# Pose-Group/FAMI-Pose

Measured on AMD Instinct MI355X. Metric: train clips/sec (5-frame 384x288 HRNet-W48), higher is better.
Workload: dtype f32

## Files before the change

### fami-pose_amd/csrc/conv.hip

```cpp
#include "common.h"
#include <type_traits>
#include <string.h>

#include "conv_epi.h"
#include "conv_pair.h"
extern "C" int fami_conv2d_fwd_bnin_ok(int N, int H, int W, int Ci, int Co);
extern "C" int fami_dcn_tune(int mode);
extern "C" int fami_bn_tune_small(long elems);
extern "C" void fami_conv_stem_tune(int on);
int fami_pair_launch(const PairCapture& c, hipStream_t s);
int fami_try_conv_stem1(int half_kind, const void* x, const void* wp, const float* bias, void* y, int N, int H, int W, int Ci, int Co,
                        int kh, int kw, int stride, int pad, int dil, int NTt, int relu, int accumulate, int out_f32, hipStream_t s,
                        const char* name, const EpiBN& epi);


struct ConvArgs {
  EpiBN e;
  int emode;
  const float* x;
  const float* wp;
  float* y;
  const float* bias;
  const float* addend;
  int N, Hi, Wi, Ci, Ho, Wo, Co;
// ... 1713 lines not shown
      for (int nt = 0; nt < NT; ++nt)
#pragma unroll
        for (int r = 0; r < 4; ++r) acc[mt][nt][r] += mine[((mt * NT + nt) * 4 + r) * 64];
  }
  if (!active) return;
  float* slabp = p.part + ((long)slab * taps + tap) * p.Ci * p.Co;
#pragma unroll
  for (int mt = 0; mt < MT; ++mt)
#pragma unroll
    for (int r = 0; r < 4; ++r) {
      const int cci = (cib * MT + mt) * 16 + kq * 4 + r;
#pragma unroll
      for (int nt = 0; nt < NT; ++nt) {
        const int cco = (cob * NT + nt) * 16 + c16;
        slabp[(long)cci * p.Co + cco] = acc[mt][nt][r];
      }
    }
}

__device__ __forceinline__ void reduce_taps_body(const float* __restrict__ part, float* __restrict__ dw, int Co, int Ci,
                                                 int taps, int psplit, int accumulate, int bid, float* sm ) {
  const long n = (long)taps * Ci * Co;
  const int o = threadIdx.x & 63, g = threadIdx.x >> 6;
  const long i = (long)bid * 64 + o;
  float s0 = 0.f, s1 = 0.f;
  if (i < n) {
    int k = g;
    for (; k + 16 < psplit; k += 32) {
      s0 += part[(long)k * n + i];
      s1 += part[(long)(k + 16) * n + i];
    }
    if (k < psplit) s0 += part[(long)k * n + i];
  }
  sm[threadIdx.x] = s0 + s1;
  __syncthreads();
  if (g == 0 && i < n) {
    float s = 0.f;
#pragma unroll
    for (int q = 0; q < 16; ++q) s += sm[q * 64 + o];
    const int co = (int)(i % Co);
    const long r = i / Co;
    const int ci = (int)(r % Ci), tap = (int)(r / Ci);
    float* d = dw + ((long)co * Ci + ci) * taps + tap;
    *d = accumulate ? *d + s : s;
  }
}
__global__ __launch_bounds__(1024) void wgrad_reduce_taps_kernel(const float* __restrict__ part,
                                                                 float* __restrict__ dw, int Co, int Ci, int taps,
                                                                 int psplit, int accumulate) {
  __shared__ float sm[1024];
  reduce_taps_body(part, dw, Co, Ci, taps, psplit, accumulate, blockIdx.x, sm);
}

__device__ __forceinline__ void reduce_taps4_body(const float* __restrict__ part, float* __restrict__ dw, int Co, int Ci,
                                                  int taps, int psplit, int accumulate, int sg, int bid, f32x4* sm ) {
  const int SG = 1 << sg, cols = 256 >> sg;
  const int o = threadIdx.x & (cols - 1), g = threadIdx.x >> (8 - sg);
  const long n4 = (long)taps * Ci * Co / 4;
  const long i = (long)bid * cols + o;
  const f32x4 z = {0.f, 0.f, 0.f, 0.f};
  f32x4 s0 = z, s1 = z, s2 = z, s3 = z;
  if (i < n4) {
    const f32x4* p4 = reinterpret_cast<const f32x4*>(part) + i;
    int k = g;
    for (; k + 7 * SG < psplit; k += 8 * SG) {
      const f32x4 v0 = p4[(long)k * n4], v1 = p4[(long)(k + SG) * n4], v2 = p4[(long)(k + 2 * SG) * n4],
                  v3 = p4[(long)(k + 3 * SG) * n4], v4 = p4[(long)(k + 4 * SG) * n4], v5 = p4[(long)(k + 5 * SG) * n4],
                  v6 = p4[(long)(k + 6 * SG) * n4], v7 = p4[(long)(k + 7 * SG) * n4];
      s0 += v0; s1 += v1; s2 += v2; s3 += v3;
      s0 += v4; s1 += v5; s2 += v6; s3 += v7;
    }
    for (; k + 3 * SG < psplit; k += 4 * SG) {
      s0 += p4[(long)k * n4];
      s1 += p4[(long)(k + SG) * n4];
      s2 += p4[(long)(k + 2 * SG) * n4];
      s3 += p4[(long)(k + 3 * SG) * n4];
    }
    for (; k < psplit; k += SG) s0 += p4[(long)k * n4];
  }
  sm[threadIdx.x] = (s0 + s1) + (s2 + s3);
  __syncthreads();
  if (g == 0 && i < n4) {
    f32x4 t = sm[o];
    for (int q = 1; q < SG; ++q) t += sm[q * cols + o];
    const long e = i * 4;
    const int co = (int)(e % Co);
    const long r = e / Co;
    const int ci = (int)(r % Ci), tap = (int)(r / Ci);
#pragma unroll
    for (int u = 0; u < 4; ++u) {
      float* d = dw + ((long)(co + u) * Ci + ci) * taps + tap;
      *d = accumulate ? *d + t[u] : t[u];
    }
  }
}
__global__ __launch_bounds__(256) void wgrad_reduce_taps4_kernel(const float* __restrict__ part, float* __restrict__ dw,
                                                                 int Co, int Ci, int taps, int psplit, int accumulate,
                                                                 int sg) {
  __shared__ f32x4 sm[256];
  reduce_taps4_body(part, dw, Co, Ci, taps, psplit, accumulate, sg, blockIdx.x, sm);
}

static void launch_reduce_taps(const float* part, float* dw, int Co, int Ci, int taps, int psplit, int accumulate,
                               hipStream_t s);

__device__ __forceinline__ void reduce_plain_body(const float* __restrict__ part, float* __restrict__ dw, long n,
                                                  int psplit, int accumulate, int bid, float* sm ) {
  const int o = threadIdx.x & 63, g = threadIdx.x >> 6;
  const long i = (long)bid * 64 + o;
  float s = 0.f;
  if (i < n)
    for (int k = g; k < psplit; k += 4) s += part[(long)k * n + i];
  sm[threadIdx.x] = s;
  __syncthreads();
  if (g == 0 && i < n) {
    s = sm[o] + sm[64 + o] + sm[128 + o] + sm[192 + o];
    dw[i] = accumulate ? dw[i] + s : s;
  }
}
__global__ __launch_bounds__(256) void wgrad_reduce_kernel(const float* __restrict__ part, float* __restrict__ dw,
                                                           long n, int psplit, int accumulate) {
  __shared__ float sm[256];
  reduce_plain_body(part, dw, n, psplit, accumulate, blockIdx.x, sm);
}

struct ReduceDesc {
  const float* part;
  float* dw;
  int Co, Ci, taps, psplit, accumulate, kind, sg, blocks;
};
#define FAMI_REDUCE_BATCH 16
struct ReduceBatch { ReduceDesc d[FAMI_REDUCE_BATCH]; };
__global__ __launch_bounds__(1024) void wgrad_reduce_batch_kernel(ReduceBatch b) {
  __shared__ f32x4 sm[256];
  const ReduceDesc& d = b.d[blockIdx.y];
  if ((int)blockIdx.x >= d.blocks) return;
  if (d.kind == 2) {
    reduce_taps_body(d.part, d.dw, d.Co, d.Ci, d.taps, d.psplit, d.accumulate, blockIdx.x, reinterpret_cast<float*>(sm));
    return;
  }
  if (threadIdx.x >= 256) return;
  if (d.kind == 1) reduce_taps4_body(d.part, d.dw, d.Co, d.Ci, d.taps, d.psplit, d.accumulate, d.sg, blockIdx.x, sm);
  else reduce_plain_body(d.part, d.dw, (long)d.Co * d.Ci * d.taps, d.psplit, d.accumulate, blockIdx.x, reinterpret_cast<float*>(sm));
}

typedef short s16x4 __attribute__((ext_vector_type(4)));
typedef __attribute__((address_space(3))) s16x4 lds_s16x4;

struct WgradLdsArgs {
  const void* x;
  const void* dy;
  float* part;
  int N, H, W, Ci, Co, P;
  int chunk;
  int nsub;
  int ciBlocks, coBlocks;
  int CiB, CoB;
  int xrow, yrow;
  int xbytes;
  int xcd;
};

template <typename H, int CIT, int COT>
__global__ __launch_bounds__(256) void conv_wgrad_h_kernel(WgradLdsArgs p) {
  typedef typename H16<H>::x8 hx8;
  extern __shared__ __attribute__((aligned(16))) char smem[];
  constexpr int NPW = (CIT * 9 + 3) / 4;
  const int tid = threadIdx.x, lane = tid & 63;
  const int wave = __builtin_amdgcn_readfirstlane(tid >> 6);
  const int l16 = lane & 15, kq = lane >> 4;
  const int rsel = l16 >> 2, piece = l16 & 3;
  int g, byl;
  xcd_tile(p.xcd, g, byl);
  const int cob = byl % p.coBlocks, cib = byl / p.coBlocks;
  const int halo = p.W + 1;
  char* xt = smem;
  char* yt = smem + p.xbytes;
  char* zrow = yt + p.chunk * p.yrow;

  int pci[NPW], ptap[NPW];
#pragma unroll
  for (int i = 0; i < NPW; ++i) {
    const int q = wave + 4 * i;
    const bool ok = q < CIT * 9;
    pci[i] = ok ? q / 9 : 0;
    ptap[i] = ok ? q % 9 : -1;
  }
  f32x4 acc[NPW][COT];
#pragma unroll
  for (int i = 0; i < NPW; ++i)
#pragma unroll
    for (int c = 0; c < COT; ++c) acc[i][c] = f32x4{0.f, 0.f, 0.f, 0.f};
  const int HW = p.H * p.W;

  for (int sub = 0; sub < p.nsub; ++sub) {
  const int p0 = (g * p.nsub + sub) * p.chunk;
// ... 267 lines not shown

template <typename T>
constexpr int storage_kind() { return std::is_same<T, float>::value ? 2 : (std::is_same<T, f16_t>::value ? 1 : 0); }

static bool wgrad_lin_ok(int H, int W, int Ci, int Co, int kh, int kw, int stride, int pad, int dil) {
  return stride == 1 && 2 * pad == dil * (kh - 1) && 2 * pad == dil * (kw - 1) && kh * kw > 1 && kh * kw <= 9 && W >= 4 &&
         Ci % 16 == 0 && Co % 16 == 0;
}
static bool geom_ok(int kh, int kw, int stride, int pad, int dil) {
  return kh >= 1 && kw >= 1 && kh <= 7 && kw <= 7 && (stride == 1 || stride == 2) && pad >= 0 && dil >= 1;
}
static inline int out_dim(int i, int k, int stride, int pad, int dil) {
  return (i + 2 * pad - dil * (k - 1) - 1) / stride + 1;
}
static int conv_args_check(const char* nm, bool ptrs, int N, int H, int W, int Ci, int Co, int kh, int kw, int stride, int pad,
                           int dil) {
  FAMI_REQUIRE(ptrs && N > 0 && H > 0 && W > 0 && Ci > 0 && Co > 0, nm, "bad argument");
  if (!geom_ok(kh, kw, stride, pad, dil)) {
    fami_set_error(nm, "unsupported geometry");
    return FAMI_ESHAPE;
  }
  return FAMI_OK;
}
template <typename Args>
static int conv_geometry(Args& a, const char* nm, int mode, int N, int H, int W, int Ci, int Co, int kh, int kw, int stride,
                         int pad, int dil, int esize, int kchunk) {
  const int Hc = out_dim(H, kh, stride, pad, dil), Wc = out_dim(W, kw, stride, pad, dil);
  a.N = N;
  a.Hi = mode ? Hc : H; a.Wi = mode ? Wc : W; a.Ci = mode ? Co : Ci;
  a.Ho = mode ? H : Hc; a.Wo = mode ? W : Wc; a.Co = mode ? Ci : Co;
  a.kh = kh; a.kw = kw; a.sh = stride == 2 ? 1 : 0; a.pad = pad; a.dil = dil;
  a.KC = fami_cdiv(a.Ci, kchunk); a.NTt = fami_cdiv(a.Co, 16);
  const long P = (long)N * a.Ho * a.Wo;
  const long xb = (long)N * a.Hi * a.Wi * a.Ci * esize, wb = (long)kh * kw * a.KC * a.NTt * 1024;
  FAMI_REQUIRE(P > 0 && P < (1L << 31) && xb < (1L << 31) && wb < (1L << 31), nm, "tensor >= 2 GiB");
  a.P = (int)P; a.x_bytes = (unsigned)xb; a.wp_bytes = (unsigned)wb;
  return FAMI_OK;
}

static thread_local ReduceDesc* g_defer = nullptr;
static ReduceDesc reduce_desc_taps(const float* part, float* dw, int Co, int Ci, int taps, int psplit, int accumulate) {
  ReduceDesc d;
  d.part = part; d.dw = dw; d.Co = Co; d.Ci = Ci; d.taps = taps; d.psplit = psplit; d.accumulate = accumulate;
  const long n = (long)Co * Ci * taps;
  if (Co % 4 == 0 && (reinterpret_cast<uintptr_t>(part) & 15) == 0) {
    int sg = 0;
    while (sg < 4 && (8 << sg) <= psplit) ++sg;
    d.kind = 1; d.sg = sg; d.blocks = fami_cdiv(n / 4, 256 >> sg);
  } else {
    d.kind = 2; d.sg = 0; d.blocks = fami_cdiv(n, 64);
  }
  return d;
}
static void launch_reduce_taps(const float* part, float* dw, int Co, int Ci, int taps, int psplit, int accumulate,
                               hipStream_t s) {
  const ReduceDesc d = reduce_desc_taps(part, dw, Co, Ci, taps, psplit, accumulate);
  if (g_defer) {
    *g_defer = d;
    return;
  }
  if (d.kind == 1)
    hipLaunchKernelGGL(wgrad_reduce_taps4_kernel, dim3(d.blocks), dim3(256), 0, s, part, dw, Co, Ci, taps, psplit, accumulate, d.sg);
  else
    hipLaunchKernelGGL(wgrad_reduce_taps_kernel, dim3(d.blocks), dim3(1024), 0, s, part, dw, Co, Ci, taps, psplit, accumulate);
}
static void launch_reduce_plain(const float* part, float* dw, int Co, int Ci, int taps, int psplit, int accumulate,
                                hipStream_t s) {
  const long n = (long)Co * Ci * taps;
  if (g_defer) {
    ReduceDesc d;
    d.part = part; d.dw = dw; d.Co = Co; d.Ci = Ci; d.taps = taps; d.psplit = psplit; d.accumulate = accumulate;
    d.kind = 0; d.sg = 0; d.blocks = fami_cdiv(n, 64);
    *g_defer = d;
    return;
  }
  hipLaunchKernelGGL(wgrad_reduce_kernel, dim3(fami_cdiv(n, 64)), dim3(256), 0, s, part, dw, n, psplit, accumulate);
}
template <typename Call>
static int with_deferred_reduce(const char* nm, long* desc_out, Call&& wgrad) {
  ReduceDesc d;
  d.part = nullptr;
  g_defer = &d;
  const int rc = wgrad();
  g_defer = nullptr;
  if (rc != FAMI_OK) return rc;
  FAMI_REQUIRE(d.part, nm, "no reduce recorded");
  memcpy(desc_out, &d, sizeof(d));
  return FAMI_OK;
}
template <typename Dgrad, typename Wgrad>
static int bwd_pair_run(const char* nm, long* desc_out, hipStream_t s, Dgrad&& dgrad, Wgrad&& wgrad) {
  PairCapture pc;
  pc.a.kind = pc.b.kind = 0;
  fami_pair_capture() = &pc;
  int rc = dgrad();
  if (rc == FAMI_OK) rc = with_deferred_reduce(nm, desc_out, wgrad);
  fami_pair_capture() = nullptr;
  if (rc != FAMI_OK) return rc;
  const int pr = fami_pair_launch(pc, s);
  FAMI_REQUIRE(pr >= 0, nm, "a recorded launch has no kernel instance");
  FAMI_CHECK_LAUNCH(nm);
  return FAMI_OK;
}

struct WgradPlan { int MT, NT, ciBlocks, coBlocks, psplit, chunk, pertap, w8; long P; };
static WgradPlan wgrad_plan(int N, int H, int W, int Ci, int Co, int kh, int kw, int stride, int pad, int dil, int w8 = 0) {
  WgradPlan q;
  const int Ho = out_dim(H, kh, stride, pad, dil), Wo = out_dim(W, kw, stride, pad, dil);
  q.P = (long)N * Ho * Wo;
  q.MT = pick_small(fami_cdiv(Ci, 16));
  q.NT = pick_small(fami_cdiv(Co, 16));
  if (g_wgrad_mt > 0 && g_wgrad_mt <= q.MT) q.MT = g_wgrad_mt;
  q.ciBlocks = fami_cdiv(fami_cdiv(Ci, 16), q.MT);
  q.coBlocks = fami_cdiv(fami_cdiv(Co, 16), q.NT);
// ... 682 lines not shown
                               epi_bwd_stats(slots, Ci, z, yrelu, mean, invstd, gamma, beta, relu));
}
template <typename HT>
static int bwd_pair_h(const char* nm, const HT* x, const HT* dy, const HT* wpd, HT* dx, float* dw, float* workspace, long ws_bytes,
                      int N, int H, int W, int Ci, int Co, int kh, int kw, int stride, int pad, int dil, int acc_dx, int acc_dw,
                      long* desc_out, const HT* z, const HT* yrelu, const float* mean, const float* invstd, const float* gamma,
                      const float* beta, int relu, void* slots, hipStream_t s) {
  FAMI_REQUIRE(desc_out, nm, "null descriptor");
  EpiBN e = epi_none();
  if (slots) {
    FAMI_REQUIRE(epi_bwd_stats_ok(z, yrelu, mean, invstd, gamma, beta, relu), nm, "bad argument");
    e = epi_bwd_stats(slots, Ci, z, yrelu, mean, invstd, gamma, beta, relu);
  }
  return bwd_pair_run(
      nm, desc_out, s,
      [&] { return conv_dgrad_h_impl<HT>(nm, dy, wpd, dx, N, H, W, Ci, Co, kh, kw, stride, pad, dil, acc_dx, s, e); },
      [&] { return wgrad_h_impl<HT>(nm, x, dy, dw, workspace, ws_bytes, N, H, W, Ci, Co, kh, kw, stride, pad, dil, acc_dw, s); });
}

extern "C" {

int fami_conv_tune(int mt, int nt, int ks) {
  g_force_mt = mt; g_force_nt = nt; g_force_ks = ks;
  return FAMI_OK;
}
int fami_conv_tune_lds(int on) {
  if (on == 9000 || on == 9001) {
    fami_conv_stem_tune(on - 9000);
    return FAMI_OK;
  }
  if (on < 0) fami_conv_stem_tune(-1);
  if (on == 10 || on == 11 || on == 20 || on == 21 || on == 30 || on == 31 || (on >= 40 && on <= 42) || (on >= 52 && on <= 54) || (on >= 60 && on <= 62) || on >= 100) {
    fami_conv_t4_tune(on);
    return FAMI_OK;
  }
  g_use_lds = on < 0 ? -1 : (on ? 1 : 0);
  g_lds_sim = on == 2;
  if (on < 0) fami_conv_t4_tune(-1);
  return FAMI_OK;
}
int fami_conv_tune_wgrad_lds(int on) {
  if (on >= 30000) {
    fami_wgrad_s3_tune(on - 30000);
    return FAMI_OK;
  }
  if (on >= 20000) {
    fami_wgrad16_tune(on - 20000);
    return FAMI_OK;
  }
  if (on >= 1000) {
    g_wgrad_ps = on - 1000;
    return FAMI_OK;
  }
  if (on >= 50 && on <= 54) {
    g_wgrad_lin = on - 50;
    return FAMI_OK;
  }
  if (on >= 100) {
    g_wgrad_mt = on - 100;
    return FAMI_OK;
  }
  if (on < 0) {
    fami_wgrad16_tune(-1);
    fami_wgrad_s3_tune(-1);
    g_wgrad_lds = 1;
    g_wgrad_lds_f32 = 2;
    g_wgrad_nsub = 2;
    g_wgrad_lin = 1;
    return FAMI_OK;
  }
  g_wgrad_lds = on ? 1 : 0;
  g_wgrad_lds_f32 = on ? 1 : 0;
  if (on > 1) g_wgrad_nsub = on - 1;
  return FAMI_OK;
}
int fami_conv_tune_xcd(int mode) {
  g_xcd = mode < 0 ? -1 : (mode & 1);
  g_xcd_w = mode < 0 ? 1 : ((mode >> 1) & 1);
  return FAMI_OK;
}
int fami_conv_tune_stages(int stages) {
  if (stages == 120 || stages == 121) {
    g_prio = stages - 120;
    return FAMI_OK;
  }
  if (stages == 110 || stages == 111) {
    g_par = stages - 110;
    return FAMI_OK;
  }
  if (stages == 100 || stages == 101) {
    g_lin_conv = stages - 100;
    return FAMI_OK;
  }
  g_stages = (stages >= 2 && stages <= 4) ? stages : 0;
  return FAMI_OK;
}
int fami_tune_reset(void) {
  fami_conv_tune(0, 0, 0);
  fami_conv_tune_lds(-1);
  fami_conv_tune_wgrad_lds(-1);
  fami_conv_tune_xcd(-1);
  g_stages = 0; g_prio = 0; g_lin_conv = 1; g_par = 1;
  g_wgrad_ps = 0; g_wgrad_mt = 0;
  fami_dcn_tune(-1);
  fami_bn_tune_small(-1);
  return FAMI_OK;
}
int fami_tune_defaults(int f32_split) {
  if (f32_split >= 0) {
    fami_conv_t4_default_split(f32_split);
    fami_wgrad_s3_default(f32_split);
  }
  return fami_tune_reset();
}

long fami_packed_weight_elems(int Co, int Ci, int kh, int kw, int mode) {
  const int kd = mode == 0 ? Ci : Co, nd = mode == 0 ? Co : Ci;
  return pack16_elems(kd, nd, kh * kw) + pack32_elems(kd, nd, kh * kw) + fami_split_image_elems(kd, nd, kh * kw);
}

int fami_pack_conv_weight_f32(const float* w_oihw, float* wp, int Co, int Ci, int kh, int kw, int mode,
// ... 77 lines not shown
  }
  if (kh == kw) {
    const long nl = fami_wgrad16_slabs(N, H, W, Ci, Co, kh, stride, pad, dil) * Co * Ci * kh * kw * (long)sizeof(float);
    if (nl > need) need = nl;
  }
  if (kh == 3 && kw == 3 && stride == 1 && pad == 1 && dil == 1) {
    const long nl = fami_wgrad_s3_slabs(N, H, W, Ci, Co) * Co * Ci * 9 * (long)sizeof(float);
    if (nl > need) need = nl;
  }
  return need;
}

int fami_conv2d_wgrad_f32(const float* x, const float* dy, float* dw, float* workspace, long ws_bytes, int N, int H,
                          int W, int Ci, int Co, int kh, int kw, int stride, int pad, int dil, int accumulate,
                          hipStream_t s) {
  return wgrad_f32_entry(x, dy, dw, workspace, ws_bytes, N, H, W, Ci, Co, kh, kw, stride, pad, dil, accumulate, s, xbn_none());
}
int fami_conv2d_wgrad_defer_f32(const float* x, const float* dy, float* dw, float* workspace, long ws_bytes, int N, int H,
                                int W, int Ci, int Co, int kh, int kw, int stride, int pad, int dil, int accumulate,
                                long* desc_out, hipStream_t s) {
  FAMI_REQUIRE(desc_out, "fami_conv2d_wgrad_defer_f32", "null descriptor");
  return with_deferred_reduce("fami_conv2d_wgrad_defer_f32", desc_out, [&] {
    return fami_conv2d_wgrad_f32(x, dy, dw, workspace, ws_bytes, N, H, W, Ci, Co, kh, kw, stride, pad, dil, accumulate, s);
  });
}
int fami_conv2d_wgrad_defer_xbn_f32(const float* z, const float* dy, float* dw, float* workspace, long ws_bytes, int N, int H,
                                    int W, int Ci, int Co, int accumulate, long* desc_out, const float* xmean,
                                    const float* xinvstd, const float* xgamma, const float* xbeta, hipStream_t s) {
  FAMI_REQUIRE(desc_out && xmean && xinvstd && xgamma && xbeta, "fami_conv2d_wgrad_defer_xbn_f32", "bad argument");
  return with_deferred_reduce("fami_conv2d_wgrad_defer_xbn_f32", desc_out, [&] {
    return wgrad_f32_entry(z, dy, dw, workspace, ws_bytes, N, H, W, Ci, Co, 3, 3, 1, 1, 1, accumulate, s,
                           xbn_wgrad(Ci, xmean, xinvstd, xgamma, xbeta));
  });
}
int fami_conv2d_bwd_pair_f32(const float* x, const float* dy, const float* wpd, float* dx, float* dw, float* workspace,
                             long ws_bytes, int N, int H, int W, int Ci, int Co, int kh, int kw, int stride, int pad, int dil,
                             int acc_dx, int acc_dw, long* desc_out, const float* xmean, const float* xinvstd,
                             const float* xgamma, const float* xbeta, hipStream_t s) {
  const char* const nm = "fami_conv2d_bwd_pair_f32";
  FAMI_REQUIRE(desc_out, nm, "null descriptor");
  XBN xb = xbn_none();
  if (xmean) {
    FAMI_REQUIRE(xinvstd && xgamma && xbeta, nm, "bad argument");
    xb = xbn_wgrad(Ci, xmean, xinvstd, xgamma, xbeta);
  }
  return bwd_pair_run(
      nm, desc_out, s,
      [&] { return conv_dgrad_f32_impl(nm, dy, wpd, nullptr, dx, N, H, W, Ci, Co, kh, kw, stride, pad, dil, acc_dx, epi_none(), s); },
      [&] { return wgrad_f32_entry(x, dy, dw, workspace, ws_bytes, N, H, W, Ci, Co, kh, kw, stride, pad, dil, acc_dw, s, xb); });
}
int fami_conv2d_xbn_ok_f32(int N, int H, int W, int Ci, int Co) {
  return (g_use_lds != 0 && fami_conv_t4_eligible_s3(N, H, W, Ci, Co) && fami_wgrad_s3_slabs(N, H, W, Ci, Co) > 0) ? 1 : 0;
}
int fami_wgrad_reduce_desc_longs(void) { return (int)((sizeof(ReduceDesc) + sizeof(long) - 1) / sizeof(long)); }
int fami_wgrad_reduce_batch(const long* descs, int n, hipStream_t s) {
  FAMI_REQUIRE(descs && n > 0, "fami_wgrad_reduce_batch", "bad argument");
  const int stride = fami_wgrad_reduce_desc_longs();
  for (int i0 = 0; i0 < n; i0 += FAMI_REDUCE_BATCH) {
    const int m = n - i0 < FAMI_REDUCE_BATCH ? n - i0 : FAMI_REDUCE_BATCH;
    ReduceBatch b;
    int maxb = 1;
    for (int i = 0; i < m; ++i) {
      memcpy(&b.d[i], descs + (long)(i0 + i) * stride, sizeof(ReduceDesc));
      if (b.d[i].blocks > maxb) maxb = b.d[i].blocks;
    }
    hipLaunchKernelGGL(wgrad_reduce_batch_kernel, dim3(maxb, m), dim3(1024), 0, s, b);
    FAMI_CHECK_LAUNCH("fami_wgrad_reduce_batch");
  }
  return FAMI_OK;
}
}

extern "C" {

long fami_packed_weight_elems_bf16(int Co, int Ci, int kh, int kw, int mode) {
  const int kd = mode == 0 ? Ci : Co, nd = mode == 0 ? Co : Ci;
  return (long)kh * kw * fami_cdiv(kd, 32) * fami_cdiv(nd, 16) * 512;
}
long fami_packed_weight_elems_f16(int Co, int Ci, int kh, int kw, int mode) {
  return fami_packed_weight_elems_bf16(Co, Ci, kh, kw, mode);
}

#define FAMI_CONV_H_ABI(sfx, HT)                                                                                       \
  int fami_conv2d_wgrad_##sfx(const HT* x, const HT* dy, float* dw, float* workspace, long ws_bytes, int N, int H,     \
                              int W, int Ci, int Co, int kh, int kw, int stride, int pad, int dil, int accumulate,     \
                              hipStream_t s) {                                                                         \
    return wgrad_h_impl<HT>("fami_conv2d_wgrad_" #sfx, x, dy, dw, workspace, ws_bytes, N, H, W, Ci, Co, kh, kw,        \
                            stride, pad, dil, accumulate, s);                                                          \
  }                                                                                                                    \
  int fami_conv2d_wgrad_defer_##sfx(const HT* x, const HT* dy, float* dw, float* workspace, long ws_bytes, int N,      \
                                    int H, int W, int Ci, int Co, int kh, int kw, int stride, int pad, int dil,        \
                                    int accumulate, long* desc_out, hipStream_t s) {                                   \
    return wgrad_defer_h<HT>("fami_conv2d_wgrad_defer_" #sfx, x, dy, dw, workspace, ws_bytes, N, H, W, Ci, Co, kh, kw, \
                             stride, pad, dil, accumulate, desc_out, s);                                               \
  }                                                                                                                    \
  int fami_pack_conv_weights_batch_##sfx(const float* params, HT* packed, const void* desc, int n, hipStream_t s) {    \
    return pack_conv_weights_batch_h<HT>("fami_pack_conv_weights_batch_" #sfx, params, packed, desc, n, s);            \
  }                                                                                                                    \
  int fami_pack_conv_weight_##sfx(const float* w_oihw, HT* wp, int Co, int Ci, int kh, int kw, int mode,               \
                                  hipStream_t s) {                                                                     \
    return pack_conv_weight_h_impl<HT>("fami_pack_conv_weight_" #sfx, w_oihw, wp, Co, Ci, kh, kw, mode, s);            \
  }                                                                                                                    \
  int fami_conv2d_fwd_##sfx(const HT* x, const HT* wp, const float* bias, void* y, int N, int H, int W, int Ci,        \
                            int Co, int kh, int kw, int stride, int pad, int dil, int relu, int accumulate,            \
                            int out_f32, hipStream_t s) {                                                              \
    return conv_fwd_h_impl<HT>("fami_conv2d_fwd_" #sfx, x, wp, bias, y, N, H, W, Ci, Co, kh, kw, stride, pad, dil,     \
                               relu, accumulate, out_f32, s);                                                          \
  }                                                                                                                    \
  int fami_conv2d_dgrad_##sfx(const HT* dy, const HT* wp, HT* dx, int N, int H, int W, int Ci, int Co, int kh,         \
                              int kw, int stride, int pad, int dil, int accumulate, hipStream_t s) {                   \
    return conv_dgrad_h_impl<HT>("fami_conv2d_dgrad_" #sfx, dy, wp, dx, N, H, W, Ci, Co, kh, kw, stride, pad, dil,     \
                                 accumulate, s);                                                                       \
  }                                                                                                                    \
  int fami_conv2d_fwd_xbn_##sfx(const HT* z, const HT* wp, const float* bias, HT* y, int N, int H, int W, int Ci,      \
                                int Co, void* slots, const float* pivot_src, const void* xslots, long xP,             \
                                const float* xgamma, const float* xbeta, float* xmean, float* xinvstd,                 \
                                float* xrunning_mean, float* xrunning_var, float xmomentum, float xeps,                \
                                hipStream_t s) {                                                                       \
    return fwd_xbn_h<HT>("fami_conv2d_fwd_xbn_" #sfx, z, wp, bias, y, N, H, W, Ci, Co, slots, pivot_src, xslots, xP,   \
// ... 45 lines not shown
```

### fami-pose_amd/csrc/route.h

```cpp
#pragma once
#include "../../include/fami_route.h"
extern "C" fami_route_t* fami_rt(void);

#define g_dcn_gather (fami_rt()->dcn_gather)
#define g_dcn_abl (fami_rt()->dcn_abl)
#define g_dcn_win_r (fami_rt()->dcn_win_r)
#define g_dcn_ksplit (fami_rt()->dcn_ksplit)
#define g_dcn_pf (fami_rt()->dcn_pf)
#define g_dcn_bwd2 (fami_rt()->dcn_bwd2)
#define g_dcn_bwd2_cap (fami_rt()->dcn_bwd2_cap)
#define g_dcn_bwd2_stage (fami_rt()->dcn_bwd2_stage)
#define g_dcn_bwd_abl (fami_rt()->dcn_bwd_abl)
#define g_dcn_bwd_scatter (fami_rt()->dcn_bwd_scatter)
#define g_prio (fami_rt()->prio)
#define g_lin_conv (fami_rt()->lin_conv)
#define g_par (fami_rt()->par)
#define g_force_mt (fami_rt()->force_mt)
#define g_force_nt (fami_rt()->force_nt)
#define g_force_ks (fami_rt()->force_ks)
#define g_stages (fami_rt()->stages)
#define g_use32 (fami_rt()->use32)
#define g_xcd_w (fami_rt()->xcd_w)
#define g_xcd (fami_rt()->xcd)
#define g_use_lds (fami_rt()->use_lds)
#define g_lds_sim (fami_rt()->lds_sim)
#define g_wgrad_nsub (fami_rt()->wgrad_nsub)
#define g_wgrad_ps (fami_rt()->wgrad_ps)
#define g_wgrad_mt (fami_rt()->wgrad_mt)
#define g_wgrad_lds (fami_rt()->wgrad_lds)
#define g_wgrad_lds_f32 (fami_rt()->wgrad_lds_f32)
#define g_wgrad_lin (fami_rt()->wgrad_lin)
#define g_stem1 (fami_rt()->stem1)
#define g_use_t4 (fami_rt()->use_t4)
#define g_t4_dil (fami_rt()->t4_dil)
#define g_use_t4_f32 (fami_rt()->use_t4_f32)
#define g_t4_bt (fami_rt()->t4_bt)
#define g_t4_s3_narrow (fami_rt()->t4_s3_narrow)
#define g_t4_s3_wdma (fami_rt()->t4_s3_wdma)
#define g_t4_s3_fill (fami_rt()->t4_s3_fill)
#define g_t4_s3_pc (fami_rt()->t4_s3_pc)
#define g_t4_s3_mt_minft (fami_rt()->t4_s3_mt_minft)
#define g_t4_s3_mt (fami_rt()->t4_s3_mt)
#define g_t4_s3_minwg (fami_rt()->t4_s3_minwg)
#define g_s3_default (fami_rt()->s3_default)
#define g_use_t4_s3 (fami_rt()->use_t4_s3)
#define g_use_t5 (fami_rt()->use_t5)
#define g_t5_rows (fami_rt()->t5_rows)
#define g_t5_maxwg (fami_rt()->t5_maxwg)
#define g_t5_h16 (fami_rt()->t5_h16)
#define g_t5_abl (fami_rt()->t5_abl)
#define g_t5_min_jobs (fami_rt()->t5_min_jobs)
#define g_t5_min_tiles (fami_rt()->t5_min_tiles)
#define g_use_t6 (fami_rt()->use_t6)
#define g_t6_rows (fami_rt()->t6_rows)
#define g_t6_min_jobs (fami_rt()->t6_min_jobs)
#define g_t6_mt (fami_rt()->t6_mt)
#define g_t7_target (fami_rt()->t7_target)
#define g_use_t7 (fami_rt()->use_t7)
#define g_t7_rows (fami_rt()->t7_rows)
#define g_t7_c64 (fami_rt()->t7_c64)
#define g_bn_in (fami_rt()->bn_in)
#define g_bwd_pair (fami_rt()->bwd_pair)
#define g_pair_wg6_target (fami_rt()->pair_wg6_target)
#define g_wg6_s2 (fami_rt()->wg6_s2)
#define g_wg6_dil (fami_rt()->wg6_dil)
#define g_wg6_c42 (fami_rt()->wg6_c42)
#define g_wg6_c4 (fami_rt()->wg6_c4)
#define g_wg6 (fami_rt()->wg6)
#define g_wg6_nu (fami_rt()->wg6_nu)
#define g_wg6_target (fami_rt()->wg6_target)
#define g_wg6_target_c4 (fami_rt()->wg6_target_c4)
#define g_wg1 (fami_rt()->wg1)
#define g_wg1_target (fami_rt()->wg1_target)
#define g_wgs (fami_rt()->wgs)
#define g_wg16_abl (fami_rt()->wg16_abl)
#define g_wg16 (fami_rt()->wg16)
#define g_wg16_bt (fami_rt()->wg16_bt)
#define g_wg16_target (fami_rt()->wg16_target)
#define g_wg16_general (fami_rt()->wg16_general)
#define g_wg16_bt18 (fami_rt()->wg16_bt18)
#define g_wgs3 (fami_rt()->wgs3)
#define g_wgs3_bt (fami_rt()->wgs3_bt)
#define g_wgs3_target (fami_rt()->wgs3_target)
#define g_wgs3_default (fami_rt()->wgs3_default)
#define g_bn_small_elems (fami_rt()->bn_small_elems)
#define g_bn2_maxg (fami_rt()->bn2_maxg)

static inline void fami_route_set_dcn_defaults(fami_route_t* q) {
  q->dcn_gather = -1;
  q->dcn_abl = 0;
  q->dcn_win_r = 0;
  q->dcn_ksplit = 1;
  q->dcn_pf = 0;
  q->dcn_bwd2 = 1;
  q->dcn_bwd2_cap = 36;
  q->dcn_bwd2_stage = 1;
  q->dcn_bwd_abl = 0;
  q->dcn_bwd_scatter = -1;
}

static inline void fami_route_set_defaults(fami_route_t* q) {
  q->size = (int)sizeof(fami_route_t);
  fami_route_set_dcn_defaults(q);
  q->prio = 0;
  q->lin_conv = 1;
  q->par = 1;
  q->force_mt = 0;
  q->force_nt = 0;
  q->force_ks = 0;
  q->stages = 0;
  q->use32 = 1;
  q->xcd_w = 1;
  q->xcd = -1;
  q->use_lds = -1;
  q->lds_sim = 0;
  q->wgrad_nsub = 2;
  q->wgrad_ps = 0;
  q->wgrad_mt = 0;
  q->wgrad_lds = 1;
  q->wgrad_lds_f32 = 2;
  q->wgrad_lin = 1;
  q->stem1 = 1;
  q->use_t4 = 1;
  q->t4_dil = 1;
  q->use_t4_f32 = 0;
  q->t4_bt = 0;
  q->t4_s3_narrow = 0;
  q->t4_s3_wdma = 1;
  q->t4_s3_fill = 2;
  q->t4_s3_pc = 0;
  q->t4_s3_mt_minft = 64;
  q->t4_s3_mt = 3;
  q->t4_s3_minwg = 0;
  q->s3_default = 1;
  q->use_t4_s3 = 1;
  q->use_t5 = 1;
  q->t5_rows = 0;
  q->t5_maxwg = 256;
  q->t5_h16 = 0;
  q->t5_abl = 0;
  q->t5_min_jobs = 200;
  q->t5_min_tiles = 0;
  q->use_t6 = 1;
  q->t6_rows = 0;
  q->t6_min_jobs = 96;
  q->t6_mt = 0;
  q->t7_target = 240;
  q->use_t7 = 1;
  q->t7_rows = 0;
  q->t7_c64 = 1;
  q->bn_in = 1;
  q->bwd_pair = 1;
  q->pair_wg6_target = 64;
  q->wg6_s2 = 1;
  q->wg6_dil = 1;
  q->wg6_c42 = 1;
  q->wg6_c4 = 1;
  q->wg6 = 1;
  q->wg6_nu = 0;
  q->wg6_target = 80;
  q->wg6_target_c4 = 160;
  q->wg1 = 1;
  q->wg1_target = 192;
  q->wgs = 1;
  q->wg16_abl = 0;
  q->wg16 = 1;
  q->wg16_bt = 0;
  q->wg16_target = 0;
  q->wg16_general = 1;
  q->wg16_bt18 = 0;
  q->wgs3 = 1;
  q->wgs3_bt = 0;
  q->wgs3_target = 0;
  q->wgs3_default = 1;
// ... 4 lines not shown
```

### include/fami.h

```cpp
#ifndef FAMI_H
#define FAMI_H
#ifdef __cplusplus
extern "C" {
#endif

typedef void* fami_stream_t;

#include "fami_route.h"
long fami_route_size(void);
int fami_route_init(fami_route_t* route);
int fami_route_bind(fami_route_t* route);

const char* fami_version(void);
const char* fami_last_error(void);
int fami_device_info(int device, int* info, char* name, int name_len);

int fami_conv_tune(int mt, int nt, int ks);
int fami_conv_tune_lds(int on);
int fami_conv_tune_wgrad_lds(int on);
int fami_conv_tune_xcd(int mode);
int fami_conv_tune_stages(int stages);
int fami_tune_reset(void);
int fami_tune_defaults(int f32_split);
int fami_conv_t5_eligible(int N, int H, int W, int Ci, int Co);
int fami_conv_t4_eligible(int N, int H, int W, int Ci, int Co);
int fami_conv_t4_s3_plan(int N, int H, int W, int Ci, int Co, int dil, int sgn, int xbn, long* out);
int fami_conv_t6_eligible(int N, int H, int W, int Ci, int Co);
long fami_packed_weight_elems(int Co, int Ci, int kh, int kw, int mode);
int fami_pack_conv_weight_f32(const float* w_oihw, float* wp, int Co, int Ci, int kh, int kw, int mode,
                              fami_stream_t stream);
int fami_pack_conv_weights_batch_f32(const float* params, float* packed, const void* desc, int n, fami_stream_t stream);
int fami_conv2d_fwd_f32(const float* x, const float* wp, const float* bias, const float* addend, float* y, int N,
                        int H, int W, int Ci, int Co, int kh, int kw, int stride, int pad, int dil, int relu,
                        int accumulate, fami_stream_t stream);
int fami_conv2d_dgrad_f32(const float* dy, const float* wp, const float* addend, float* dx, int N, int H, int W,
                          int Ci, int Co, int kh, int kw, int stride, int pad, int dil, int accumulate,
                          fami_stream_t stream);
int fami_conv2d_fwd_stats_f32(const float* x, const float* wp, const float* bias, float* y, int N, int H, int W, int Ci,
                              int Co, int kh, int kw, int stride, int pad, int dil, void* slots, const float* pivot_src,
                              fami_stream_t stream);
int fami_conv2d_dgrad_bnstats_f32(const float* dy, const float* wp, float* dx, int N, int H, int W, int Ci, int Co,
                                  int kh, int kw, int stride, int pad, int dil, int accumulate, const float* z,
                                  const float* yrelu, const float* mean, const float* invstd, const float* gamma,
                                  const float* beta, int relu, void* slots, fami_stream_t stream);
long fami_conv2d_wgrad_workspace(int N, int H, int W, int Ci, int Co, int kh, int kw, int stride, int pad, int dil);
int fami_wgrad_reduce_desc_longs(void);
int fami_wgrad_reduce_batch(const long* descs, int n, fami_stream_t stream);
int fami_conv2d_wgrad_defer_f32(const float* x, const float* dy, float* dw, float* workspace, long ws_bytes, int N,
                                int H, int W, int Ci, int Co, int kh, int kw, int stride, int pad, int dil,
                                int accumulate, long* desc_out, fami_stream_t stream);
int fami_conv2d_wgrad_f32(const float* x, const float* dy, float* dw, float* workspace, long ws_bytes, int N, int H,
                          int W, int Ci, int Co, int kh, int kw, int stride, int pad, int dil, int accumulate,
                          fami_stream_t stream);

long fami_bn_workspace(int C);
int fami_bn_stats_f32(const float* x, long P, int C, float* mean, float* invstd, float* running_mean,
                      float* running_var, float momentum, float eps, float* ws, fami_stream_t stream);
int fami_bn_train_fwd_f32(const float* x, const float* residual, float* y, const float* gamma, const float* beta,
                          float* mean, float* invstd, float* running_mean, float* running_var, long P, int C,
                          int relu, float momentum, float eps, float* ws, fami_stream_t stream);
int fami_bn_running_update_f32(float* running_mean, float* running_var, const float* mean, const float* invstd, int C,
                               long P, float momentum, float eps, fami_stream_t stream);
int fami_bn_running_update_batch_f32(const long* ptrs, const float* meta, int n, fami_stream_t stream);
int fami_bn_eval_stats_f32(const float* running_mean, const float* running_var, float* mean, float* invstd, int C,
                           float eps, fami_stream_t stream);
int fami_bn_apply_f32(const float* x, const float* mean, const float* invstd, const float* gamma, const float* beta,
                      const float* residual, float* y, long P, int C, int relu, fami_stream_t stream);
int fami_bn_bwd_f32(const float* dy, const float* x, const float* y, const float* mean, const float* invstd,
                    const float* gamma, float* dx, float* dgamma, float* dbeta, float* dres, long P, int C, int relu,
                    int acc_dx, int acc_param, int acc_dres, float* ws, fami_stream_t stream);
int fami_bn_eval_bwd_f32(const float* dy, const float* x, const float* y, const float* mean,
                     const float* invstd, const float* gamma, float* dx, float* dgamma, float* dbeta,
                     float* dres, long P, int C, int relu, int acc_dx, int acc_param, int acc_dres, float* ws,
                     fami_stream_t stream);
long fami_bn_slots_bytes(int C);
int fami_bn_train_fwd2_f32(const float* x, const float* residual, float* y, const float* gamma, const float* beta,
                           float* mean, float* invstd, float* running_mean, float* running_var, long P, int C,
                           int relu, float momentum, float eps, void* slots, fami_stream_t stream);
int fami_bn_bwd2_f32(const float* dy, const float* x, const float* y, const float* mean, const float* invstd,
                     const float* gamma, const float* beta, float* dx, float* dgamma, float* dbeta, float* dres, long P,
                     int C, int relu, int acc_dx, int acc_param, int acc_dres, void* slots, fami_stream_t stream);
int fami_bn_is_small(long P, int C);
int fami_conv2d_xbn_ok(int N, int H, int W, int Ci, int Co);
int fami_conv2d_fwd_bnin_ok(int N, int H, int W, int Ci, int Co);
int fami_conv2d_bwd_pair_ok(int N, int H, int W, int Ci, int Co, int kh, int kw, int stride, int pad, int dil);
int fami_conv2d_bwd_pair_key(int N, int H, int W, int Ci, int Co, int* out);
int fami_conv2d_bwd_pair_ok_f32(int N, int H, int W, int Ci, int Co, int kh, int kw, int stride, int pad, int dil);
int fami_conv2d_bwd_pair_key_f32(int N, int H, int W, int Ci, int Co, int* out);
int fami_conv2d_bwd_pair_f32(const float* x, const float* dy, const float* wpd, float* dx, float* dw, float* workspace,
                             long ws_bytes, int N, int H, int W, int Ci, int Co, int kh, int kw, int stride, int pad, int dil,
                             int acc_dx, int acc_dw, long* desc_out, const float* xmean, const float* xinvstd,
                             const float* xgamma, const float* xbeta, fami_stream_t stream);
int fami_conv2d_xbn_ok_f32(int N, int H, int W, int Ci, int Co);
int fami_conv2d_fwd_xbn_f32(const float* z, const float* wp, const float* bias, float* y, int N, int H, int W, int Ci,
                            int Co, void* slots, const float* pivot_src, const void* xslots, long xP,
                            const float* xgamma, const float* xbeta, float* xmean, float* xinvstd,
                            float* xrunning_mean, float* xrunning_var, float xmomentum, float xeps, fami_stream_t stream);
int fami_conv2d_wgrad_defer_xbn_f32(const float* z, const float* dy, float* dw, float* workspace, long ws_bytes, int N,
                                    int H, int W, int Ci, int Co, int accumulate, long* desc_out, const float* xmean,
// ... 486 lines not shown
```

### include/fami_route.h

```cpp
#ifndef FAMI_ROUTE_H
#define FAMI_ROUTE_H
#ifdef __cplusplus
extern "C" {
#endif

typedef struct fami_route_t {
  int size;
  int  dcn_gather;
  int  dcn_abl;
  int  dcn_win_r;
  int  dcn_ksplit;
  int  dcn_pf;
  int  dcn_bwd2;
  int  dcn_bwd2_cap;
  int  dcn_bwd2_stage;
  int  dcn_bwd_abl;
  int  dcn_bwd_scatter;
  int  prio;
  int  lin_conv;
  int  par;
  int  force_mt;
  int  force_nt;
  int  force_ks;
  int  stages;
  int  use32;
  int  xcd_w;
  int  xcd;
  int  use_lds;
  int  lds_sim;
  int  wgrad_nsub;
  int  wgrad_ps;
  int  wgrad_mt;
  int  wgrad_lds;
  int  wgrad_lds_f32;
  int  wgrad_lin;
  int  stem1;
  int  use_t4;
  int  t4_dil;
  int  use_t4_f32;
  int  t4_bt;
  int  t4_s3_narrow;
  int  t4_s3_wdma;
  int  t4_s3_fill;
  int  t4_s3_pc;
  int  t4_s3_mt_minft;
  int  t4_s3_mt;
  int  t4_s3_minwg;
  int  s3_default;
  int  use_t4_s3;
  int  use_t5;
  int  t5_rows;
  int  t5_maxwg;
  int  t5_h16;
  int  t5_abl;
  int  t5_min_jobs;
  int  t5_min_tiles;
  int  use_t6;
  int  t6_rows;
  int  t6_min_jobs;
  int  t6_mt;
  int  t7_target;
  int  use_t7;
  int  t7_rows;
  int  t7_c64;
  int  bn_in;
  int  bwd_pair;
  int  pair_wg6_target;
  int  wg6_s2;
  int  wg6_dil;
  int  wg6_c42;
  int  wg6_c4;
  int  wg6;
  int  wg6_nu;
  int  wg6_target;
  int  wg6_target_c4;
  int  wg1;
  int  wg1_target;
  int  wgs;
  int  wg16_abl;
  int  wg16;
  int  wg16_bt;
  int  wg16_target;
  int  wg16_general;
  int  wg16_bt18;
  int  wgs3;
  int  wgs3_bt;
  int  wgs3_target;
  int  wgs3_default;
// ... 9 lines not shown
```

Measured before the change: 92.17.

## Add LDS-transposed tiled wgrad reduction with coalesced row stores and flat batch grid

```diff
diff --git a/fami-pose_amd/csrc/conv.hip b/fami-pose_amd/csrc/conv.hip
--- a/fami-pose_amd/csrc/conv.hip
+++ b/fami-pose_amd/csrc/conv.hip
@@ -1789,6 +1789,27 @@
   reduce_taps_body(part, dw, Co, Ci, taps, psplit, accumulate, blockIdx.x, sm);
 }
 
+__device__ __forceinline__ f32x4 reduce_quad_group(const f32x4* __restrict__ p4, long n4, int psplit, int g, int SG) {
+  const f32x4 z = {0.f, 0.f, 0.f, 0.f};
+  f32x4 s0 = z, s1 = z, s2 = z, s3 = z;
+  int k = g;
+  for (; k + 7 * SG < psplit; k += 8 * SG) {
+    const f32x4 v0 = p4[(long)k * n4], v1 = p4[(long)(k + SG) * n4], v2 = p4[(long)(k + 2 * SG) * n4],
+                v3 = p4[(long)(k + 3 * SG) * n4], v4 = p4[(long)(k + 4 * SG) * n4], v5 = p4[(long)(k + 5 * SG) * n4],
+                v6 = p4[(long)(k + 6 * SG) * n4], v7 = p4[(long)(k + 7 * SG) * n4];
+    s0 += v0; s1 += v1; s2 += v2; s3 += v3;
+    s0 += v4; s1 += v5; s2 += v6; s3 += v7;
+  }
+  for (; k + 3 * SG < psplit; k += 4 * SG) {
+    s0 += p4[(long)k * n4];
+    s1 += p4[(long)(k + SG) * n4];
+    s2 += p4[(long)(k + 2 * SG) * n4];
+    s3 += p4[(long)(k + 3 * SG) * n4];
+  }
+  for (; k < psplit; k += SG) s0 += p4[(long)k * n4];
+  return (s0 + s1) + (s2 + s3);
+}
+
 __device__ __forceinline__ void reduce_taps4_body(const float* __restrict__ part, float* __restrict__ dw, int Co, int Ci,
                                                   int taps, int psplit, int accumulate, int sg, int bid, f32x4* sm ) {
   const int SG = 1 << sg, cols = 256 >> sg;
@@ -1796,26 +1817,7 @@
   const long n4 = (long)taps * Ci * Co / 4;
   const long i = (long)bid * cols + o;
   const f32x4 z = {0.f, 0.f, 0.f, 0.f};
-  f32x4 s0 = z, s1 = z, s2 = z, s3 = z;
-  if (i < n4) {
-    const f32x4* p4 = reinterpret_cast<const f32x4*>(part) + i;
-    int k = g;
-    for (; k + 7 * SG < psplit; k += 8 * SG) {
-      const f32x4 v0 = p4[(long)k * n4], v1 = p4[(long)(k + SG) * n4], v2 = p4[(long)(k + 2 * SG) * n4],
-                  v3 = p4[(long)(k + 3 * SG) * n4], v4 = p4[(long)(k + 4 * SG) * n4], v5 = p4[(long)(k + 5 * SG) * n4],
-                  v6 = p4[(long)(k + 6 * SG) * n4], v7 = p4[(long)(k + 7 * SG) * n4];
-      s0 += v0; s1 += v1; s2 += v2; s3 += v3;
-      s0 += v4; s1 += v5; s2 += v6; s3 += v7;
-    }
-    for (; k + 3 * SG < psplit; k += 4 * SG) {
-      s0 += p4[(long)k * n4];
-      s1 += p4[(long)(k + SG) * n4];
-      s2 += p4[(long)(k + 2 * SG) * n4];
-      s3 += p4[(long)(k + 3 * SG) * n4];
-    }
-    for (; k < psplit; k += SG) s0 += p4[(long)k * n4];
-  }
-  sm[threadIdx.x] = (s0 + s1) + (s2 + s3);
+  sm[threadIdx.x] = i < n4 ? reduce_quad_group(reinterpret_cast<const f32x4*>(part) + i, n4, psplit, g, SG) : z;
   __syncthreads();
   if (g == 0 && i < n4) {
     f32x4 t = sm[o];
@@ -1836,6 +1838,63 @@
                                                                  int sg) {
   __shared__ f32x4 sm[256];
   reduce_taps4_body(part, dw, Co, Ci, taps, psplit, accumulate, sg, blockIdx.x, sm);
+}
+
+#define FAMI_ROWS_THREADS 576
+#define FAMI_ROWS_LDS 2560
+struct ReduceTile { int ct, it, nco, blocks, threads; };
+__device__ __forceinline__ void reduce_rows4_body(const float* __restrict__ part, float* __restrict__ dw, int Co, int Ci,
+                                                  int taps, int psplit, int accumulate, int sg, ReduceTile tl, int bid,
+                                                  float* sm ) {
+  const int SG = 1 << sg;
+  const int co0 = (bid % tl.nco) * tl.ct, ci0 = (bid / tl.nco) * tl.it;
+  const int cte = tl.ct < Co - co0 ? tl.ct : Co - co0, ite = tl.it < Ci - ci0 ? tl.it : Ci - ci0;
+  const int ctq = cte >> 2, run = ite * taps, cs = run | 1, gs = cte * cs, Q = run * ctq;
+  const int t = threadIdx.x;
+  if (t < Q * SG) {
+    const int g = t / Q, q = t - g * Q;
+    const int cq = q % ctq, r = q / ctq;
+    const int cil = r % ite, tap = r / ite;
+    const long n4 = (long)taps * Ci * Co / 4;
+    const long i = ((long)tap * Ci + ci0 + cil) * (Co >> 2) + (co0 >> 2) + cq;
+    const f32x4 v = reduce_quad_group(reinterpret_cast<const f32x4*>(part) + i, n4, psplit, g, SG);
+    float* d = sm + g * gs + cq * 4 * cs + cil * taps + tap;
+    d[0] = v[0]; d[cs] = v[1]; d[2 * cs] = v[2]; d[3 * cs] = v[3];
+  }
+  __syncthreads();
+  const int nt = blockDim.x;
+  const long rowlen = (long)Ci * taps;
+  float* d0 = dw + ((long)co0 * Ci + ci0) * taps;
+  if ((run & 3) == 0 && (rowlen & 3) == 0 && (reinterpret_cast<uintptr_t>(d0) & 15) == 0) {
+    const int rq = run >> 2;
+    for (int e = t; e < cte * rq; e += nt) {
+      const int col = e / rq, j = (e - col * rq) * 4;
+      const float* s = sm + col * cs + j;
+      f32x4 v = {s[0], s[1], s[2], s[3]};
+      for (int g = 1; g < SG; ++g) {
+        s += gs;
+        const f32x4 a = {s[0], s[1], s[2], s[3]};
+        v += a;
+      }
+      f32x4* d = reinterpret_cast<f32x4*>(d0 + col * rowlen + j);
+      *d = accumulate ? *d + v : v;
+    }
+  } else {
+    for (int e = t; e < cte * run; e += nt) {
+      const int col = e / run, j = e - col * run;
+      const float* s = sm + col * cs + j;
+      float v = s[0];
+      for (int g = 1; g < SG; ++g) v += s[g * gs];
+      float* d = d0 + col * rowlen + j;
+      *d = accumulate ? *d + v : v;
+    }
+  }
+}
+__global__ __launch_bounds__(FAMI_ROWS_THREADS) void wgrad_reduce_rows4_kernel(const float* __restrict__ part,
+                                                                               float* __restrict__ dw, int Co, int Ci, int taps,
+                                                                               int psplit, int accumulate, int sg, ReduceTile tl) {
+  __shared__ float sm[FAMI_ROWS_LDS];
+  reduce_rows4_body(part, dw, Co, Ci, taps, psplit, accumulate, sg, tl, blockIdx.x, sm);
 }
 
 static void launch_reduce_taps(const float* part, float* dw, int Co, int Ci, int taps, int psplit, int accumulate,
@@ -1867,18 +1926,35 @@
   int Co, Ci, taps, psplit, accumulate, kind, sg, blocks;
 };
 #define FAMI_REDUCE_BATCH 16
-struct ReduceBatch { ReduceDesc d[FAMI_REDUCE_BATCH]; };
-__global__ __launch_bounds__(1024) void wgrad_reduce_batch_kernel(ReduceBatch b) {
-  __shared__ f32x4 sm[256];
-  const ReduceDesc& d = b.d[blockIdx.y];
-  if ((int)blockIdx.x >= d.blocks) return;
+struct ReduceBatch {
+  ReduceDesc d[FAMI_REDUCE_BATCH];
+  ReduceTile t[FAMI_REDUCE_BATCH];
+  int start[FAMI_REDUCE_BATCH + 1];
+  int m;
+};
+__global__ __launch_bounds__(1024) __attribute__((amdgpu_waves_per_eu(8))) void wgrad_reduce_batch_kernel(ReduceBatch b) {
+  __shared__ __attribute__((aligned(16))) float sm[FAMI_ROWS_LDS];
+  int e = blockIdx.y, bid = blockIdx.x;
+  if (b.m > 0) {
+    e = 0;
+    while (e + 1 < b.m && bid >= b.start[e + 1]) ++e;
+    bid -= b.start[e];
+  }
+  const ReduceDesc& d = b.d[e];
+  const ReduceTile tl = b.t[e];
+  if (tl.threads > 0) {
+    if (bid >= tl.blocks) return;
+    reduce_rows4_body(d.part, d.dw, d.Co, d.Ci, d.taps, d.psplit, d.accumulate, d.sg, tl, bid, sm);
+    return;
+  }
+  if (bid >= d.blocks) return;
   if (d.kind == 2) {
-    reduce_taps_body(d.part, d.dw, d.Co, d.Ci, d.taps, d.psplit, d.accumulate, blockIdx.x, reinterpret_cast<float*>(sm));
+    reduce_taps_body(d.part, d.dw, d.Co, d.Ci, d.taps, d.psplit, d.accumulate, bid, sm);
     return;
   }
   if (threadIdx.x >= 256) return;
-  if (d.kind == 1) reduce_taps4_body(d.part, d.dw, d.Co, d.Ci, d.taps, d.psplit, d.accumulate, d.sg, blockIdx.x, sm);
-  else reduce_plain_body(d.part, d.dw, (long)d.Co * d.Ci * d.taps, d.psplit, d.accumulate, blockIdx.x, reinterpret_cast<float*>(sm));
+  if (d.kind == 1) reduce_taps4_body(d.part, d.dw, d.Co, d.Ci, d.taps, d.psplit, d.accumulate, d.sg, bid, reinterpret_cast<f32x4*>(sm));
+  else reduce_plain_body(d.part, d.dw, (long)d.Co * d.Ci * d.taps, d.psplit, d.accumulate, bid, sm);
 }
 
 typedef short s16x4 __attribute__((ext_vector_type(4)));
@@ -2252,6 +2328,35 @@
   }
   return d;
 }
+static ReduceTile reduce_rows_plan(int Co, int Ci, int taps, int psplit) {
+  ReduceTile t = {0, 0, 0, 0, 0};
+  if (Co < 4 || Co % 4 != 0 || Ci < 1 || taps < 1 || psplit < 1) return t;
+  int sg = 0;
+  while (sg < 4 && (8 << sg) <= psplit) ++sg;
+  if (sg > 1) return t;
+  const int SG = 1 << sg, coq = Co / 4;
+  int it = 36 / taps;
+  it = it < 1 ? 1 : (it > Ci ? Ci : it);
+  int room = FAMI_ROWS_THREADS / (taps * it * SG);
+  if (room > 16) room = 16;
+  if (room > coq) room = coq;
+  if (room < 1) return t;
+  int ctq = room;
+  while (coq % ctq != 0) --ctq;
+  if (2 * ctq <= room) ctq = room;
+  if (ctq < 4 && ctq < coq) return t;
+  if ((long)SG * ctq * 4 * ((it * taps) | 1) > FAMI_ROWS_LDS) return t;
+  const long blocks = (long)fami_cdiv(coq, ctq) * fami_cdiv(Ci, it);
+  if (blocks >= (1L << 24)) return t;
+  t.ct = ctq * 4; t.it = it; t.nco = fami_cdiv(coq, ctq); t.blocks = (int)blocks;
+  t.threads = (taps * it * ctq * SG + 63) / 64 * 64;
+  return t;
+}
+static ReduceTile reduce_tile_of(const ReduceDesc& d) {
+  if (d.kind == 1 && g_wgrad_rows == 1) return reduce_rows_plan(d.Co, d.Ci, d.taps, d.psplit);
+  const ReduceTile none = {0, 0, 0, 0, 0};
+  return none;
+}
 static void launch_reduce_taps(const float* part, float* dw, int Co, int Ci, int taps, int psplit, int accumulate,
                                hipStream_t s) {
   const ReduceDesc d = reduce_desc_taps(part, dw, Co, Ci, taps, psplit, accumulate);
@@ -2259,7 +2364,10 @@
     *g_defer = d;
     return;
   }
-  if (d.kind == 1)
+  const ReduceTile tl = reduce_tile_of(d);
+  if (tl.threads > 0)
+    hipLaunchKernelGGL(wgrad_reduce_rows4_kernel, dim3(tl.blocks), dim3(tl.threads), 0, s, part, dw, Co, Ci, taps, psplit, accumulate, d.sg, tl);
+  else if (d.kind == 1)
     hipLaunchKernelGGL(wgrad_reduce_taps4_kernel, dim3(d.blocks), dim3(256), 0, s, part, dw, Co, Ci, taps, psplit, accumulate, d.sg);
   else
     hipLaunchKernelGGL(wgrad_reduce_taps_kernel, dim3(d.blocks), dim3(1024), 0, s, part, dw, Co, Ci, taps, psplit, accumulate);
@@ -3048,6 +3156,10 @@
     g_wgrad_ps = on - 1000;
     return FAMI_OK;
   }
+  if (on >= 60 && on <= 62) {
+    g_wgrad_rows = on - 60;
+    return FAMI_OK;
+  }
   if (on >= 50 && on <= 54) {
     g_wgrad_lin = on - 50;
     return FAMI_OK;
@@ -3063,6 +3175,7 @@
     g_wgrad_lds_f32 = 2;
     g_wgrad_nsub = 2;
     g_wgrad_lin = 1;
+    g_wgrad_rows = 1;
     return FAMI_OK;
   }
   g_wgrad_lds = on ? 1 : 0;
@@ -3246,6 +3359,19 @@
 int fami_conv2d_xbn_ok_f32(int N, int H, int W, int Ci, int Co) {
   return (g_use_lds != 0 && fami_conv_t4_eligible_s3(N, H, W, Ci, Co) && fami_wgrad_s3_slabs(N, H, W, Ci, Co) > 0) ? 1 : 0;
 }
+long fami_wgrad_s3_slab_count(int N, int H, int W, int Ci, int Co) { return fami_wgrad_s3_slabs(N, H, W, Ci, Co); }
+int fami_wgrad_reduce_plan(int Co, int Ci, int taps, int psplit, int* out) {
+  ReduceDesc d;
+  d.Co = Co; d.Ci = Ci; d.taps = taps; d.psplit = psplit;
+  d.kind = (Co > 0 && Co % 4 == 0) ? 1 : 2;
+  const ReduceTile t = reduce_tile_of(d);
+  if (out) {
+    int sg = 0;
+    while (sg < 4 && (8 << sg) <= psplit) ++sg;
+    out[0] = t.ct; out[1] = t.it; out[2] = t.nco; out[3] = t.blocks; out[4] = t.threads; out[5] = d.kind == 1 ? sg : 0;
+  }
+  return t.threads > 0 ? 1 : 0;
+}
 int fami_wgrad_reduce_desc_longs(void) { return (int)((sizeof(ReduceDesc) + sizeof(long) - 1) / sizeof(long)); }
 int fami_wgrad_reduce_batch(const long* descs, int n, hipStream_t s) {
   FAMI_REQUIRE(descs && n > 0, "fami_wgrad_reduce_batch", "bad argument");
@@ -3253,12 +3379,25 @@
   for (int i0 = 0; i0 < n; i0 += FAMI_REDUCE_BATCH) {
     const int m = n - i0 < FAMI_REDUCE_BATCH ? n - i0 : FAMI_REDUCE_BATCH;
     ReduceBatch b;
-    int maxb = 1;
+    int maxb = 1, threads = 256;
+    long total = 0;
     for (int i = 0; i < m; ++i) {
       memcpy(&b.d[i], descs + (long)(i0 + i) * stride, sizeof(ReduceDesc));
-      if (b.d[i].blocks > maxb) maxb = b.d[i].blocks;
-    }
-    hipLaunchKernelGGL(wgrad_reduce_batch_kernel, dim3(maxb, m), dim3(1024), 0, s, b);
+      b.t[i] = reduce_tile_of(b.d[i]);
+      const int nb = b.t[i].threads > 0 ? b.t[i].blocks : b.d[i].blocks;
+      const int nt = b.t[i].threads > 0 ? b.t[i].threads : (b.d[i].kind == 2 ? 1024 : 256);
+      FAMI_REQUIRE(nb > 0, "fami_wgrad_reduce_batch", "bad descriptor");
+      if (nb > maxb) maxb = nb;
+      if (nt > threads) threads = nt;
+      b.start[i] = (int)total;
+      total += nb;
+    }
+    for (int i = m; i <= FAMI_REDUCE_BATCH; ++i) b.start[i] = (int)total;
+    for (int i = m; i < FAMI_REDUCE_BATCH; ++i) b.t[i] = b.t[0], b.d[i] = b.d[0];
+    FAMI_REQUIRE(total < (1L << 31), "fami_wgrad_reduce_batch", "too many blocks");
+    b.m = g_wgrad_rows != 0 ? m : 0;
+    if (b.m > 0) hipLaunchKernelGGL(wgrad_reduce_batch_kernel, dim3((unsigned)total), dim3(threads), 0, s, b);
+    else hipLaunchKernelGGL(wgrad_reduce_batch_kernel, dim3(maxb, m), dim3(1024), 0, s, b);
     FAMI_CHECK_LAUNCH("fami_wgrad_reduce_batch");
   }
   return FAMI_OK;
diff --git a/fami-pose_amd/csrc/route.h b/fami-pose_amd/csrc/route.h
--- a/fami-pose_amd/csrc/route.h
+++ b/fami-pose_amd/csrc/route.h
@@ -30,6 +30,7 @@
 #define g_wgrad_lds (fami_rt()->wgrad_lds)
 #define g_wgrad_lds_f32 (fami_rt()->wgrad_lds_f32)
 #define g_wgrad_lin (fami_rt()->wgrad_lin)
+#define g_wgrad_rows (fami_rt()->wgrad_rows)
 #define g_stem1 (fami_rt()->stem1)
 #define g_use_t4 (fami_rt()->use_t4)
 #define g_t4_dil (fami_rt()->t4_dil)
@@ -120,6 +121,7 @@
   q->wgrad_lds = 1;
   q->wgrad_lds_f32 = 2;
   q->wgrad_lin = 1;
+  q->wgrad_rows = 1;
   q->stem1 = 1;
   q->use_t4 = 1;
   q->t4_dil = 1;
diff --git a/include/fami.h b/include/fami.h
--- a/include/fami.h
+++ b/include/fami.h
@@ -45,6 +45,8 @@
                                   const float* beta, int relu, void* slots, fami_stream_t stream);
 long fami_conv2d_wgrad_workspace(int N, int H, int W, int Ci, int Co, int kh, int kw, int stride, int pad, int dil);
 int fami_wgrad_reduce_desc_longs(void);
+int fami_wgrad_reduce_plan(int Co, int Ci, int taps, int psplit, int* out);
+long fami_wgrad_s3_slab_count(int N, int H, int W, int Ci, int Co);
 int fami_wgrad_reduce_batch(const long* descs, int n, fami_stream_t stream);
 int fami_conv2d_wgrad_defer_f32(const float* x, const float* dy, float* dw, float* workspace, long ws_bytes, int N,
                                 int H, int W, int Ci, int Co, int kh, int kw, int stride, int pad, int dil,
diff --git a/include/fami_route.h b/include/fami_route.h
--- a/include/fami_route.h
+++ b/include/fami_route.h
@@ -34,6 +34,7 @@
   int  wgrad_lds;
   int  wgrad_lds_f32;
   int  wgrad_lin;
+  int  wgrad_rows;
   int  stem1;
   int  use_t4;
   int  t4_dil;
```

Measured after the change: 92.65 (median of 6 runs). Within noise of the previous version (+0.5%).
